# TongkunGuan/CCD

Measured on AMD Instinct MI355X. Metric: images/sec (32x128 crops, 2 views) CCD-ViT-Small pretrain step, higher is better.
Workload: dtype bf16; 1 GPU; CCD_pretrain_vit_small bf16, bs=256/GPU, 2 views 32x128, out_dim=65536, drop_path 0.1, dataset-mask branch (pseudo-epoch 1), synthetic batch in HBM; global_batch=256, parallelism=dp1

## Files before the change

### ccd_amd/csrc/abi_impl.h

```cpp
#pragma once

#include "../../include/ccd_hip.h"
#include "kernels/common.h"
#include "kernels/gemm.h"
#include "kernels/gemm256.h"
#include "kernels/gemm_row384.h"
#include "kernels/mlp_fused.h"
#include "kernels/rowgemm.h"
#include "kernels/mlp_bwd.h"
#include "kernels/rowproj.h"
#include "kernels/attention_fwd.h"
#include "kernels/attention_probs.h"
#include "kernels/attention_bwd.h"
#include "kernels/attention_bwd1.h"
#include "kernels/gemm_tn384.h"
#include "kernels/layernorm.h"
#include "kernels/charmap.h"
#include "kernels/cluster.h"
#include "kernels/ssim.h"
#include "kernels/datapipe.h"
#include "kernels/embed.h"
#include "kernels/head.h"
#include "kernels/loss.h"
#include "kernels/headloss.h"
#include "kernels/optim.h"
#include "kernels/conv.h"
#include "kernels/cls_tail.h"
#include "kernels/decoder.h"
#include "kernels/decoder_xattn.h"

#define CCD_CHECK(cond, code) \
    do {                      \
        if (!(cond)) return (code); \
    } while (0)
#define CCD_ALIGNED16(p) ((((uintptr_t)(p)) & 15u) == 0)
#define CCD_MAX_OPERAND_BYTES 0x7ffffff0L

static int ccd_grid_cus(long tiles = 0);
static int ccd_gemm_grid(ccd::GemmParams& p, int tiles, int splits) {
    p.work_items = tiles * splits;
    const int cap = 2 * ccd_grid_cus((p.work_items + 1) / 2);
    return p.work_items < cap ? p.work_items : cap;
}

template <bool TN>
static int ccd_launch_gemm(ccd::GemmParams p, int epilogue, int splits, void* stream) {
    const int tiles = ((p.M + ccd::GEMM_BM - 1) / ccd::GEMM_BM) * ((p.N + ccd::GEMM_BN - 1) / ccd::GEMM_BN);
    const dim3 grid(ccd_gemm_grid(p, tiles, splits)), block(256);
    const size_t smem = ccd::GEMM_SMEM_BYTES;
    switch (epilogue) {
        case CCD_EPI_BF16: CCD_LAUNCH((ccd::gemm_bf16_kernel<TN, ccd::EPI_BF16>), grid, block, smem, stream, p); break;
        case CCD_EPI_GELU: CCD_LAUNCH((ccd::gemm_bf16_kernel<TN, ccd::EPI_GELU>), grid, block, smem, stream, p); break;
        case CCD_EPI_RESID: CCD_LAUNCH((ccd::gemm_bf16_kernel<TN, ccd::EPI_RESID>), grid, block, smem, stream, p); break;
        case CCD_EPI_F32: CCD_LAUNCH((ccd::gemm_bf16_kernel<TN, ccd::EPI_F32>), grid, block, smem, stream, p); break;
        case CCD_EPI_ATOMIC: CCD_LAUNCH((ccd::gemm_bf16_kernel<TN, ccd::EPI_ATOMIC>), grid, block, smem, stream, p); break;
        case CCD_EPI_DGELU: CCD_LAUNCH((ccd::gemm_bf16_kernel<TN, ccd::EPI_DGELU>), grid, block, smem, stream, p); break;
        default: return CCD_EINVAL;
    }
    return ccd_rt_last_error();
}

static unsigned ccd_stream_blocks(long total, int per_thread) {
    long blocks = (total + 256L * per_thread - 1) / (256L * per_thread);
    const long cap = 16L * ccd_rt_num_cus();
    if (blocks > cap) blocks = cap;
    return (unsigned)(blocks < 1 ? 1 : blocks);
}
static void ccd_reduce_geometry(long rows, int N, int* cgn_log2, int* col_blocks, int* rows_per_block, int* row_blocks) {
    int lg = 0;
    while (lg < 5 && (8 << lg) < N) ++lg;
    const int cgn = 1 << lg, rln = ccd::COLSUM_THREADS >> lg;
    *cgn_log2 = lg;
    *col_blocks = (N + 8 * cgn - 1) / (8 * cgn);
    long rb = (rows * (long)(16 * cgn) + (1L << 17) - 1) / (1L << 17);
    const long cap = (2L * ccd_rt_num_cus() + *col_blocks - 1) / *col_blocks;
    if (rb > cap) rb = cap;
    if (rb < 1) rb = 1;
    long rpb = (rows + rb - 1) / rb;
    rpb = ((rpb + rln - 1) / rln) * rln;
    *rows_per_block = (int)rpb;
    *row_blocks = (int)((rows + rpb - 1) / rpb);
}
struct CcdPolicy {
    int gemm_256 = 1;
    int gemm_256_min_m = 2048, gemm_256_min_n = 384;
    int gemm_256_f32 = 0;
    int gemm_256_deep = 0;
    int gemm_row384 = 0;
    int rowproj = 1;
    int rowproj_min_m = 16384;
    int rowproj_rb = 0;
    int rowgemm = 1;
    int ln_bwd_bpc = 5;
    int dec_attn_simt = 0;
    int attn_tr = 1;
    int attn_onepass = 1;
    int attn_skew = 0;
    int gemm_tn384 = 1;
    int gemm_tn384_geom = 0;
    int gemm_tn384_min_tiles = 6;
    int cu_reserve = 0;
    int cu_reserve_window = -1;
    int cu_reserve_left = 0;
    int rowgemm_adma = 1;
    int tn_ws = 1;
    int lab = 0;
};
struct CcdPolicyKey { const char* name; int CcdPolicy::*field; };
static const CcdPolicyKey ccd_policy_keys[] = {
    {"gemm_256", &CcdPolicy::gemm_256}, {"gemm_256_min_m", &CcdPolicy::gemm_256_min_m},
    {"gemm_256_min_n", &CcdPolicy::gemm_256_min_n}, {"gemm_256_f32", &CcdPolicy::gemm_256_f32},
    {"gemm_256_deep", &CcdPolicy::gemm_256_deep}, {"gemm_row384", &CcdPolicy::gemm_row384},
    {"rowproj", &CcdPolicy::rowproj}, {"rowproj_min_m", &CcdPolicy::rowproj_min_m}, {"rowproj_rb", &CcdPolicy::rowproj_rb},
    {"rowgemm", &CcdPolicy::rowgemm}, {"ln_bwd_bpc", &CcdPolicy::ln_bwd_bpc}, {"dec_attn_simt", &CcdPolicy::dec_attn_simt}, {"attn_onepass", &CcdPolicy::attn_onepass}, {"attn_skew", &CcdPolicy::attn_skew}, {"attn_tr", &CcdPolicy::attn_tr}, {"gemm_tn384", &CcdPolicy::gemm_tn384}, {"gemm_tn384_min_tiles", &CcdPolicy::gemm_tn384_min_tiles}, {"gemm_tn384_geom", &CcdPolicy::gemm_tn384_geom}, {"cu_reserve", &CcdPolicy::cu_reserve}, {"cu_reserve_window", &CcdPolicy::cu_reserve_window}, {"cu_reserve_left", &CcdPolicy::cu_reserve_left}, {"rowgemm_adma", &CcdPolicy::rowgemm_adma}, {"tn_ws", &CcdPolicy::tn_ws}, {"lab", &CcdPolicy::lab}};
static CcdPolicy& ccd_policy() {
    static CcdPolicy pol = [] {
        CcdPolicy q;
        for (const CcdPolicyKey& k : ccd_policy_keys) {
            char env[64] = "CCD_";
            size_t n = 4;
            for (const char* c = k.name; *c && n + 1 < sizeof(env); ++c) env[n++] = (char)(*c >= 'a' && *c <= 'z' ? *c - 32 : *c);
            env[n] = 0;
            if (const char* v = getenv(env)) q.*(k.field) = atoi(v);
        }
        return q;
    }();
    return pol;
}
static int ccd_grid_cus(long tiles) {
    CcdPolicy& pol = ccd_policy();
    int reserve = pol.cu_reserve;
    if (reserve > 0 && pol.cu_reserve_window >= 0) {
        if (pol.cu_reserve_left > 0) --pol.cu_reserve_left;
        else reserve = 0;
    }
    const int all = ccd_rt_num_cus();
    if (reserve > 0 && tiles > 0 && 8 * reserve <= all) {
        const long full = (tiles + all - 1) / all, less = (tiles + (all - reserve) - 1) / (all - reserve);
        if (less > full && full <= 4) reserve = 0;
    }
    const int cus = all - reserve;
    return cus > 1 ? cus : 1;
}
static bool ccd_rowproj_takes(const ccd::GemmParams& p, int epilogue) {
    const CcdPolicy& pol = ccd_policy();
    return pol.rowproj && epilogue == CCD_EPI_BF16 && (p.K == 384 || p.K == 512) && p.N % 64 == 0 && p.N <= 4096 &&
           p.M >= pol.rowproj_min_m && !p.d_rows && !p.colsum && p.alpha == 1.0f && p.ldc % 8 == 0 &&
           ccd::rp_smem_bytes(p.K, p.N) <= 160 * 1024 &&
           ((long)p.M + 512) * p.lda * 2 < CCD_MAX_OPERAND_BYTES && ((long)p.M + 512) * p.ldc * 2 < CCD_MAX_OPERAND_BYTES;
}
static int ccd_launch_rowproj(const ccd::GemmParams& p, void* stream) {
    ccd::RowProjParams q;
    q.a = reinterpret_cast<const ccd::bf16_t*>(p.A); q.lda = p.lda; q.w = reinterpret_cast<const ccd::bf16_t*>(p.B); q.ldw = p.ldb;
    q.bias = p.bias; q.out = reinterpret_cast<ccd::bf16_t*>(p.C); q.ldc = p.ldc; q.M = p.M; q.N = p.N;
    const int cus = ccd_grid_cus((p.M + ccd::rp_rows(p.K == 384 ? 2 : 1) - 1) / ccd::rp_rows(p.K == 384 ? 2 : 1)), smem = ccd::rp_smem_bytes(p.K, p.N);
    if (p.K == 384) {
        const int tiles = (p.M + ccd::rp_rows(2) - 1) / ccd::rp_rows(2), rb = ccd_policy().rowproj_rb;
        if (rb == 1 || (rb == 0 && tiles < cus)) {
            const int tiles1 = (p.M + ccd::rp_rows(1) - 1) / ccd::rp_rows(1);
            CCD_LAUNCH((ccd::rowproj_kernel<384, 1>), dim3(tiles1 < cus ? tiles1 : cus), dim3(ccd::RP_THREADS), smem, stream, q);
        } else {
            CCD_LAUNCH((ccd::rowproj_kernel<384, 2>), dim3(tiles < cus ? tiles : cus), dim3(ccd::RP_THREADS), smem, stream, q);
        }
    } else {
        const int tiles = (p.M + ccd::rp_rows(1) - 1) / ccd::rp_rows(1);
        CCD_LAUNCH((ccd::rowproj_kernel<512, 1>), dim3(tiles < cus ? tiles : cus), dim3(ccd::RP_THREADS), smem, stream, q);
    }
    return ccd_rt_last_error();
}
template <int BN, bool DEEP = false>
static int ccd_launch_gemm256(const ccd::GemmParams& p, int epilogue, void* stream) {
    const int tiles = ((p.M + ccd::G256_BM - 1) / ccd::G256_BM) * ((p.N + BN - 1) / BN);
    const int cus = ccd_grid_cus();
    const dim3 grid(tiles < cus ? tiles : cus), block(ccd::G256_THREADS);
    const size_t smem = ccd::g256_smem_bytes(p.N, p.colsum != nullptr);
    switch (epilogue) {
        case CCD_EPI_BF16: CCD_LAUNCH((ccd::gemm256_kernel<ccd::EPI_BF16, BN, DEEP>), grid, block, smem, stream, p); break;
        case CCD_EPI_GELU: CCD_LAUNCH((ccd::gemm256_kernel<ccd::EPI_GELU, BN, DEEP>), grid, block, smem, stream, p); break;
        case CCD_EPI_RESID: CCD_LAUNCH((ccd::gemm256_kernel<ccd::EPI_RESID, BN, DEEP>), grid, block, smem, stream, p); break;
        case CCD_EPI_F32: CCD_LAUNCH((ccd::gemm256_kernel<ccd::EPI_F32, BN, DEEP>), grid, block, smem, stream, p); break;
        case CCD_EPI_DGELU: CCD_LAUNCH((ccd::gemm256_kernel<ccd::EPI_DGELU, BN, DEEP>), grid, block, smem, stream, p); break;
        default: return CCD_EINVAL;
    }
    return ccd_rt_last_error();
}
static int ccd_launch_gemm_row384(const ccd::GemmParams& p, int epilogue, void* stream, int cus = -1) {
    const int tiles = (p.M + ccd::GR_BM - 1) / ccd::GR_BM;
    if (cus < 0) cus = ccd_grid_cus(tiles);
    const dim3 grid(tiles < cus ? tiles : cus), block(ccd::GR_THREADS);
    const size_t smem = ccd::GR_SMEM_BYTES;
    switch (epilogue) {
        case CCD_EPI_BF16: CCD_LAUNCH((ccd::gemm_row384_kernel<ccd::EPI_BF16>), grid, block, smem, stream, p); break;
        case CCD_EPI_RESID: CCD_LAUNCH((ccd::gemm_row384_kernel<ccd::EPI_RESID>), grid, block, smem, stream, p); break;
        case CCD_EPI_F32: CCD_LAUNCH((ccd::gemm_row384_kernel<ccd::EPI_F32>), grid, block, smem, stream, p); break;
        case 7: CCD_LAUNCH((ccd::gemm_row384_kernel<ccd::EPI_RESID_LN>), grid, block, smem, stream, p); break;
        case 8: CCD_LAUNCH((ccd::gemm_row384_kernel<ccd::EPI_LNBWD>), grid, block, smem, stream, p); break;
        default: return CCD_EINVAL;
    }
    return ccd_rt_last_error();
}

template <int WM, int WN, int STAGES, int TI, int TJ>
static int ccd_launch_tn384_geom(ccd::GemmParams& p, int Mc, float* ws, long ws_floats, void* stream) {
    using G = ccd::Tn3Geom<WM, WN, STAGES, TI, TJ>;
    const int per_cu = 8 / G::WAVES;
    const int t1 = (p.M / G::TP) * (p.N / G::TQ), t2 = (p.M2 / G::TP) * (p.N2 / G::TQ), slots = per_cu * ccd_grid_cus();
    const int xcds = slots >= 8 * (t1 > t2 ? t1 : t2) ? 8 : 1;
    const int spx = slots / xcds;
    int s1 = 0, s2 = 0;
    unsigned long long units1 = 0, units2 = 0;
    for (int x = 0; x < xcds; ++x) {
        int rem = spx, u1 = 0, u2 = 0;
        while (true) {
            const bool first = t2 == 0 || s1 < s2 || (s1 == s2 && t1 >= t2);
            if (first && t1 <= rem && u1 < 255) { ++u1; ++s1; rem -= t1; }
            else if (!first && t2 <= rem && u2 < 255) { ++u2; ++s2; rem -= t2; }
            else if (first && t2 > 0 && s2 <= s1 && t2 <= rem && u2 < 255) { ++u2; ++s2; rem -= t2; }
            else if (!first && s1 <= s2 && t1 <= rem && u1 < 255) { ++u1; ++s1; rem -= t1; }
            else break;
        }
        units1 |= (unsigned long long)u1 << (8 * x);
        units2 |= (unsigned long long)u2 << (8 * x);
    }
    if (s1 < 1 || (t2 > 0 && s2 < 1)) return CCD_ESHAPE;
    auto rows_per = [&](int& slices) {
        int per = (Mc + slices - 1) / slices;
        per = ((per + ccd::TN3_BK - 1) / ccd::TN3_BK) * ccd::TN3_BK;
        slices = (Mc + per - 1) / per;
        return per;
    };
    p.k_per_split = rows_per(s1); p.work_items = s1;
    if (t2 > 0) { p.per2 = rows_per(s2); p.slices2 = s2; }
    p.units1 = units1; p.units2 = units2; p.m_fastest = xcds;
    const long need1 = (long)s1 * p.M * p.N, need2 = t2 > 0 ? (long)s2 * p.M2 * p.N2 : 0;
    const bool use_ws = ws && need1 + need2 <= ws_floats && (s1 > 1 || s2 > 1) && p.ldc % 4 == 0 && (t2 == 0 || p.ldc2 % 4 == 0) &&
                        !(p.rps_shift & 1);
    p.ws = use_ws ? ws : nullptr;
    p.ws2 = use_ws ? ws + need1 : nullptr;
    CCD_LAUNCH((ccd::gemm_tn384_kernel<WM, WN, STAGES, TI, TJ>), dim3(xcds * spx), dim3(G::THREADS), G::SMEM_BYTES, stream, p);
    if (use_ws) {
        ccd::Tn3ReduceParams r;
        r.ws[0] = p.ws; r.ws[1] = p.ws2; r.C[0] = reinterpret_cast<float*>(p.C); r.C[1] = reinterpret_cast<float*>(p.C2);
        r.ldc[0] = p.ldc; r.ldc[1] = p.ldc2; r.S[0] = s1; r.S[1] = t2 > 0 ? s2 : 0; r.P[0] = p.M; r.P[1] = t2 > 0 ? p.M2 : 0;
        r.Q[0] = p.N; r.Q[1] = t2 > 0 ? p.N2 : 0; r.alpha = p.alpha;
        const long n4 = ((long)p.M * p.N + (t2 > 0 ? (long)p.M2 * p.N2 : 0)) / 4;
        CCD_LAUNCH(ccd::tn3_reduce_kernel, dim3((unsigned)((n4 + 255) / 256)), dim3(256), 0, stream, r);
    }
    return ccd_rt_last_error();
}

extern "C" {

int ccd_abi_version(void) { return 16; }
const char* ccd_build_info(void) { return "ccd_hip gfx950 bf16-mfma abi16"; }
int ccd_policy_set(const char* key, int value) {
    CCD_CHECK(key, CCD_EINVAL);
    for (const CcdPolicyKey& k : ccd_policy_keys)
        if (!strcmp(k.name, key)) { ccd_policy().*(k.field) = value; return CCD_OK; }
    return CCD_EINVAL;
}
int ccd_policy_get(const char* key, int* value) {
    CCD_CHECK(key && value, CCD_EINVAL);
    for (const CcdPolicyKey& k : ccd_policy_keys)
        if (!strcmp(k.name, key)) { *value = ccd_policy().*(k.field); return CCD_OK; }
    return CCD_EINVAL;
}

int ccd_gemm_nt(const ccd_bf16* A, long lda, const ccd_bf16* B, long ldb, int M, int N, int K, int epilogue, void* C,
                long ldc, void* C2, long ldc2, const float* bias, const float* resid, long ldr,
                const float* rowscale, int rows_per_sample, const ccd_bf16* aux, long ldaux, float alpha,
                int m_fastest, const int* d_rows, int rows_mul, float* colsum, void* stream) {
    CCD_CHECK(A && B && (C || (epilogue == CCD_EPI_GELU && C2)), CCD_EINVAL);
    CCD_CHECK(CCD_ALIGNED16(A) && CCD_ALIGNED16(B) && CCD_ALIGNED16(C), CCD_EINVAL);
    CCD_CHECK(!colsum || epilogue == CCD_EPI_BF16 || epilogue == CCD_EPI_DGELU, CCD_EINVAL);
    if (M == 0 || N == 0) return CCD_OK;
    CCD_CHECK(M > 0 && N > 0 && K > 0, CCD_EINVAL);
    CCD_CHECK(K % 64 == 0 && N % 8 == 0 && lda % 8 == 0 && ldb % 8 == 0 && ldc % 4 == 0, CCD_ESHAPE);
    CCD_CHECK(((long)M * lda + K) * 2 < CCD_MAX_OPERAND_BYTES && ((long)N * ldb + K) * 2 < CCD_MAX_OPERAND_BYTES, CCD_ESHAPE);
    CCD_CHECK(epilogue != CCD_EPI_GELU || (C2 && ldc2 % 8 == 0), CCD_EINVAL);
    CCD_CHECK(epilogue != CCD_EPI_RESID || (resid && ldr % 4 == 0 && rows_per_sample > 0), CCD_EINVAL);
    CCD_CHECK(epilogue != CCD_EPI_DGELU || (aux && ldaux % 8 == 0 && (!C2 || ldc2 % 8 == 0)), CCD_EINVAL);
    ccd::GemmParams p = ccd::GemmParams();
    p.A = A; p.B = B; p.lda = lda; p.ldb = ldb; p.M = M; p.N = N; p.K = K;
    p.C = C; p.ldc = ldc; p.C2 = C2; p.ldc2 = ldc2; p.bias = bias; p.resid = resid; p.ldr = ldr;
    p.rowscale = rowscale; p.rows_per_sample = rows_per_sample; p.aux = aux; p.ldaux = ldaux;
    p.rps_shift = -1;
    if (rows_per_sample > 0 && (rows_per_sample & (rows_per_sample - 1)) == 0)
        for (int sft = 0; sft < 31; ++sft) if ((1 << sft) == rows_per_sample) p.rps_shift = sft;
    p.k_per_split = K; p.m_fastest = m_fastest; p.alpha = alpha; p.d_rows = d_rows; p.rows_mul = rows_mul;
    p.colsum = colsum;
    const CcdPolicy& pol = ccd_policy();
    if (ccd_rowproj_takes(p, epilogue)) return ccd_launch_rowproj(p, stream);
    if (pol.gemm_row384 >= 1 && N <= ccd::GR_BN && M >= pol.gemm_256_min_m &&
        (epilogue == CCD_EPI_RESID || epilogue == CCD_EPI_F32 || (epilogue == CCD_EPI_BF16 && pol.gemm_row384 >= 2)))
        return ccd_launch_gemm_row384(p, epilogue, stream);
    const bool bf16_out = epilogue == CCD_EPI_BF16 || epilogue == CCD_EPI_GELU || epilogue == CCD_EPI_DGELU;
    const bool f32_256 = epilogue != CCD_EPI_ATOMIC && (pol.gemm_256_f32 || N % 256 == 0);
    const bool colsum_fits = !colsum || N <= ccd::G256_MAX_COLSUM_N;
    const bool dgelu_fits = epilogue != CCD_EPI_DGELU || (((long)M + 256) * ldaux * 2 < CCD_MAX_OPERAND_BYTES &&
        ((long)M + 256) * ldc * 2 < CCD_MAX_OPERAND_BYTES && (!C2 || ((long)M + 256) * ldc2 * 2 < CCD_MAX_OPERAND_BYTES));
    if (pol.gemm_256 >= 1 && (bf16_out || f32_256) && M >= pol.gemm_256_min_m &&
        N >= pol.gemm_256_min_n && colsum_fits && dgelu_fits) {
        if (pol.gemm_256_deep) return ccd_launch_gemm256<256, true>(p, epilogue, stream);
        return ccd_launch_gemm256<256>(p, epilogue, stream);
    }
    if (pol.gemm_256 >= 2 && epilogue != CCD_EPI_ATOMIC && M >= pol.gemm_256_min_m && colsum_fits && dgelu_fits) return ccd_launch_gemm256<128>(p, epilogue, stream);
    int splits = 1;
    if (epilogue == CCD_EPI_ATOMIC && K >= 16384) {
        p.k_per_split = 8192;
        splits = (K + 8191) / 8192;
    }
    return ccd_launch_gemm<false>(p, epilogue, splits, stream);
}

int ccd_gemm_nt_resid_ln(const ccd_bf16* A, long lda, const ccd_bf16* B, long ldb, int M, int N, int K, float* C, long ldc,
                         const float* bias, const float* resid, long ldr, const float* rowscale, int rows_per_sample,
                         const float* ln_gamma, const float* ln_beta, float ln_eps, ccd_bf16* y, long ldy, float* mean,
                         float* rstd, void* stream) {
    CCD_CHECK(A && B && C && resid && ln_gamma && ln_beta && y && mean && rstd, CCD_EINVAL);
    CCD_CHECK(CCD_ALIGNED16(A) && CCD_ALIGNED16(B) && CCD_ALIGNED16(C) && CCD_ALIGNED16(resid) && CCD_ALIGNED16(y), CCD_EINVAL);
    if (M == 0) return CCD_OK;
    CCD_CHECK(M > 0 && N > 0 && K > 0 && rows_per_sample > 0, CCD_EINVAL);
    CCD_CHECK(N <= 512 && N % 8 == 0 && K % 64 == 0 && lda % 8 == 0 && ldb % 8 == 0 && ldc % 4 == 0 && ldr % 4 == 0 &&
              ldy % 8 == 0, CCD_ESHAPE);
    CCD_CHECK(((long)M * lda + K) * 2 < CCD_MAX_OPERAND_BYTES && ((long)N * ldb + K) * 2 < CCD_MAX_OPERAND_BYTES, CCD_ESHAPE);
    const int cus = ccd_grid_cus((M + ccd::RG_BM - 1) / ccd::RG_BM);
    if (ccd_policy().rowgemm && (N == 512 || ccd_policy().rowgemm == 2) && (N == 128 || N == 256 || N == 384 || N == 512) &&
        K % (64 * ccd::rg_ring(N)) == 0 &&
        ((long)M + (long)cus * ccd::RG_BM) * lda * 2 < CCD_MAX_OPERAND_BYTES && (long)M * ldr * 4 < CCD_MAX_OPERAND_BYTES &&
        (long)M * ldc * 4 < CCD_MAX_OPERAND_BYTES) {
        ccd::RowGemmParams q = ccd::RowGemmParams();
        q.A = A; q.lda = lda; q.W = B; q.ldw = ldb; q.M = M; q.K = K; q.gamma = ln_gamma; q.ln_beta = ln_beta; q.ln_eps = ln_eps;
        q.bias = bias; q.resid = resid; q.ldr = ldr; q.out = C; q.ldc = ldc; q.ln_y = y; q.ld_y = ldy; q.ln_mean = mean;
        q.ln_rstd = rstd; q.rowscale = rowscale; q.rows_per_sample = rows_per_sample; q.lab = ccd_policy().lab;
        const int tiles = (M + ccd::RG_BM - 1) / ccd::RG_BM, smem = ccd::rg_smem_bytes(N);
        const dim3 grid(tiles < cus ? tiles : cus), block(ccd::RG_THREADS);
        if (N == 512) CCD_LAUNCH((ccd::rowgemm_kernel<512, ccd::rg_ring(512), ccd::RG_RESID_LN>), grid, block, smem, stream, q);
        else if (N == 384 && ccd_policy().rowgemm_adma)
            CCD_LAUNCH((ccd::rowgemm_kernel<384, 3, ccd::RG_RESID_LN, true>), grid, block, ccd::rg_smem_bytes_adma(384), stream, q);
        else if (N == 384) CCD_LAUNCH((ccd::rowgemm_kernel<384, ccd::rg_ring(384), ccd::RG_RESID_LN>), grid, block, smem, stream, q);
        else if (N == 256) CCD_LAUNCH((ccd::rowgemm_kernel<256, ccd::rg_ring(256), ccd::RG_RESID_LN>), grid, block, smem, stream, q);
        else CCD_LAUNCH((ccd::rowgemm_kernel<128, ccd::rg_ring(128), ccd::RG_RESID_LN>), grid, block, smem, stream, q);
        return ccd_rt_last_error();
    }
    CCD_CHECK(N <= ccd::GR_BN, CCD_ESHAPE);
    ccd::GemmParams p = ccd::GemmParams();
    p.A = A; p.B = B; p.lda = lda; p.ldb = ldb; p.M = M; p.N = N; p.K = K; p.C = C; p.ldc = ldc; p.bias = bias;
    p.resid = resid; p.ldr = ldr; p.rowscale = rowscale; p.rows_per_sample = rows_per_sample; p.alpha = 1.0f; p.rows_mul = 1;
    p.k_per_split = K;
    p.rps_shift = -1;
    for (int sft = 0; sft < 31; ++sft) if ((1 << sft) == rows_per_sample) p.rps_shift = sft;
    p.ln_gamma = ln_gamma; p.ln_beta = ln_beta; p.ln_eps = ln_eps; p.ln_y = y; p.ld_y = ldy; p.ln_mean = mean; p.ln_rstd = rstd;
    return ccd_launch_gemm_row384(p, 7 , stream, cus);
}

struct CcdLnTap {
    const ccd_bf16* tap_dy = nullptr;
    long ld_tap = 0;
    const float* tap_gamma = nullptr;
    float* tap_dgamma = nullptr;
    float* tap_dbeta = nullptr;
};
static int ccd_gemm_nt_lnbwd_any(const ccd_bf16* A, long lda, const ccd_bf16* B, long ldb, int M, int N, int K, const float* x, long ldx,
                                 const float* mean, const float* rstd, const float* gamma, void* g, int g16, long ldg, int accumulate,
                                 float* dgamma, float* dbeta, ccd_bf16* gb, long ldgb, const float* rowscale, int rows_per_sample,
                                 float* dbias, void* stream, const CcdLnTap& tap = CcdLnTap()) {
    if (tap.tap_dy) {
        CCD_CHECK(tap.tap_gamma && tap.tap_dgamma && tap.tap_dbeta && CCD_ALIGNED16(tap.tap_dy) && tap.ld_tap % 8 == 0, CCD_EINVAL);
        CCD_CHECK(g16 && N == 384 && ccd_policy().rowgemm && K % (64 * ccd::rg_ring(N)) == 0 && (long)M * tap.ld_tap * 2 < CCD_MAX_OPERAND_BYTES,
                  CCD_ESHAPE);
    }
    CCD_CHECK(A && B && x && mean && rstd && gamma && g && dgamma && dbeta, CCD_EINVAL);
    CCD_CHECK(CCD_ALIGNED16(A) && CCD_ALIGNED16(B) && CCD_ALIGNED16(x) && CCD_ALIGNED16(g) && CCD_ALIGNED16(gb), CCD_EINVAL);
    if (M == 0) return CCD_OK;
    CCD_CHECK(M > 0 && N > 0 && K > 0 && (!rowscale || rows_per_sample > 0), CCD_EINVAL);
    CCD_CHECK(N <= 512 && N % 8 == 0 && K % 64 == 0 && lda % 8 == 0 && ldb % 8 == 0 && ldx % 4 == 0 && ldg % 4 == 0 &&
              (!gb || ldgb % 4 == 0), CCD_ESHAPE);
    CCD_CHECK(((long)M * lda + K) * 2 < CCD_MAX_OPERAND_BYTES && ((long)N * ldb + K) * 2 < CCD_MAX_OPERAND_BYTES, CCD_ESHAPE);
    const int cus = ccd_grid_cus((M + ccd::RG_BM - 1) / ccd::RG_BM);
    if (ccd_policy().rowgemm && (N == 128 || N == 256 || N == 384 || N == 512) && K % (64 * ccd::rg_ring(N)) == 0 && ldg % 4 == 0 &&
        ((long)M + (long)cus * ccd::RG_BM) * lda * 2 < CCD_MAX_OPERAND_BYTES && (long)M * ldx * 4 < CCD_MAX_OPERAND_BYTES &&
        (long)M * ldg * 4 < CCD_MAX_OPERAND_BYTES && (!g16 || (N <= 384 && ldg % 8 == 0))) {
        ccd::RowGemmParams q;
        q.A = A; q.lda = lda; q.W = B; q.ldw = ldb; q.M = M; q.K = K; q.x = x; q.ldx = ldx; q.mean = mean; q.rstd = rstd;
        q.gamma = gamma; q.g = g; q.ldg = ldg; q.accumulate = accumulate; q.dgamma = dgamma; q.dbeta = dbeta; q.gb = gb;
        q.ld_gb = ldgb; q.rowscale = gb ? rowscale : nullptr; q.rows_per_sample = rows_per_sample > 0 ? rows_per_sample : 1;
        q.dbias = gb ? dbias : nullptr; q.lab = ccd_policy().lab;
        q.bias = nullptr; q.resid = nullptr; q.out = nullptr; q.ln_beta = nullptr; q.ln_y = nullptr; q.ln_mean = q.ln_rstd = nullptr;
        q.ldr = q.ldc = q.ld_y = 0; q.ln_eps = 0.f;
        q.tap_dy = tap.tap_dy; q.ld_tap = tap.ld_tap; q.tap_gamma = tap.tap_gamma; q.tap_dgamma = tap.tap_dgamma; q.tap_dbeta = tap.tap_dbeta;
        const int tiles = (M + ccd::RG_BM - 1) / ccd::RG_BM, smem = ccd::rg_smem_bytes(N);
        const dim3 grid(tiles < cus ? tiles : cus), block(ccd::RG_THREADS);
// ... 1356 lines not shown
```

### ccd_amd/csrc/kernels/gemm_tn384.h

```cpp
#pragma once

namespace ccd {

constexpr int TN3_BK = 32;
template <int WM, int WN, int STAGES_, int TI_ = 3, int TJ_ = 3>
struct Tn3Geom {
    static constexpr int WAVES = WM * WN, THREADS = 64 * WAVES, STAGES = STAGES_, TI = TI_, TJ = TJ_;
    static constexpr int TP = 32 * TI * WM, TQ = 32 * TJ * WN;
    static constexpr int A_ROWB = TP * 2, B_ROWB = TQ * 2;
    static constexpr int A_BYTES = TN3_BK * A_ROWB, B_BYTES = TN3_BK * B_ROWB, STAGE_BYTES = A_BYTES + B_BYTES;
    static constexpr int SMEM_BYTES = STAGES * STAGE_BYTES;
    static constexpr int A_PIECES = A_BYTES / 1024 / WAVES;
    static constexpr int B_TOTAL = B_BYTES / 1024;
    static constexpr int B_PIECES = (B_TOTAL + WAVES - 1) / WAVES;
    static constexpr int B_FULL = B_TOTAL - (B_PIECES - 1) * WAVES;
    static constexpr int PER_STAGE = A_PIECES + B_PIECES;
    static_assert((TI == 3 && TJ == 3) || (TI == 4 && TJ == 2), "the two hand-scheduled stage bodies below");
    static_assert(A_BYTES % (1024 * WAVES) == 0 && (PER_STAGE == 5 || PER_STAGE == 6), "piece schedule below");
};
template <int ROWB>
__device__ __forceinline__ int tn3_swz(int row) {
    static_assert(ROWB % 256 == 0 || ROWB % 256 == 128, "");
    return ROWB % 256 == 0 ? (row & 3) << 2 : ((row >> 1) & 1) << 2;
}

template <int WM, int WN, int STAGES, int TI = 3, int TJ = 3>
__global__ __launch_bounds__(64 * WM * WN, 8 / (WM * WN)) void gemm_tn384_kernel(GemmParams p) {
    using G = Tn3Geom<WM, WN, STAGES, TI, TJ>;
    constexpr int AHEAD = STAGES - 1;
    char* smem = dynamic_smem();
    const int t = threadIdx.x, lane = t & 63, w = t >> 6, hf = lane >> 5, lq = lane & 31;
    const int wm = w % WM, wn = w / WM;
    const int tiles1 = (p.M / G::TP) * (p.N / G::TQ), tiles2 = (p.M2 / G::TP) * (p.N2 / G::TQ);
    const int xcds = p.m_fastest, xcd = (int)blockIdx.x % xcds, slot = (int)blockIdx.x / xcds;
    const int u1 = (int)((p.units1 >> (8 * xcd)) & 255ull), u2 = (int)((p.units2 >> (8 * xcd)) & 255ull);
    int base1 = 0, base2 = 0;
    for (int y = 0; y < xcd; ++y) {
        base1 += (int)((p.units1 >> (8 * y)) & 255ull);
        base2 += (int)((p.units2 >> (8 * y)) & 255ull);
    }
    int tile, slice;
    if (slot < u1 * tiles1) {
        tile = slot % tiles1;
        slice = base1 + slot / tiles1;
    } else {
        const int s2 = slot - u1 * tiles1;
        if (s2 >= u2 * tiles2) return;
        tile = s2 % tiles2;
        slice = base2 + s2 / tiles2;
        p.A = p.A2; p.B = p.B2; p.lda = p.lda2; p.ldb = p.ldb2; p.M = p.M2; p.N = p.N2; p.C = p.C2; p.ldc = p.ldc2;
        p.k_per_split = p.per2; p.work_items = p.slices2; p.ws = p.ws2;
    }
    if (slice >= p.work_items) return;
    const int tiles_q = p.N / G::TQ;
    const int p0 = (tile / tiles_q) * G::TP, q0 = (tile % tiles_q) * G::TQ;
    const int k_begin = slice * p.k_per_split;
    const int k_end = k_begin + p.k_per_split < p.K ? k_begin + p.k_per_split : p.K;
    const int nk = k_end > k_begin ? (k_end - k_begin) / TN3_BK : 0;
    if (nk == 0) return;

    const bf16_t* ga[G::A_PIECES];
    const bf16_t* gb[G::B_PIECES];
#pragma unroll
    for (int i = 0; i < G::A_PIECES; ++i) {
        const int byte = 1024 * (G::A_PIECES * w + i) + 16 * lane;
        const int row = byte / G::A_ROWB, pos = (byte % G::A_ROWB) >> 4;
        ga[i] = p.A + (long)(k_begin + row) * p.lda + p0 + (pos ^ tn3_swz<G::A_ROWB>(row)) * 8;
    }
#pragma unroll
    for (int i = 0; i < G::B_PIECES; ++i) {
        const int byte = 1024 * (w + G::WAVES * i) + 16 * lane;
        const int row = (byte / G::B_ROWB) & (TN3_BK - 1), pos = (byte % G::B_ROWB) >> 4;
        gb[i] = p.B + (long)(k_begin + row) * p.ldb + q0 + (pos ^ tn3_swz<G::B_ROWB>(row)) * 8;
    }
    const long a_step = (long)TN3_BK * p.lda, b_step = (long)TN3_BK * p.ldb;
    const bool b_last = w < G::B_FULL;
    auto dma_piece = [&](int s, int i) {
        char* base = smem + (s % STAGES) * G::STAGE_BYTES;
        if (i < G::A_PIECES) {
            stream_glds16<NT_TN>(ga[i], base + (G::A_PIECES * w + i) * 1024);
            ga[i] += a_step;
        } else {
            const int ib = i - G::A_PIECES;
            if (ib < G::B_PIECES - 1 || b_last) {
                stream_glds16<NT_TN>(gb[ib], base + G::A_BYTES + (w + G::WAVES * ib) * 1024);
                gb[ib] += b_step;
            }
        }
    };
    auto dma = [&](int s) {
#pragma unroll
        for (int i = 0; i < G::PER_STAGE; ++i) dma_piece(s, i);
    };
    auto wait_steps = [&](int in_flight) {
        if (b_last) {
            if (in_flight >= 3) glds_wait<3 * G::PER_STAGE>();
            else if (in_flight == 2) glds_wait<2 * G::PER_STAGE>();
            else if (in_flight == 1) glds_wait<G::PER_STAGE>();
            else glds_wait_all();
        } else {
            if (in_flight >= 3) glds_wait<3 * (G::PER_STAGE - 1)>();
            else if (in_flight == 2) glds_wait<2 * (G::PER_STAGE - 1)>();
            else if (in_flight == 1) glds_wait<G::PER_STAGE - 1>();
            else glds_wait_all();
        }
    };

    const int j = lane & 15, g16 = (lane >> 4) & 1, r4 = j >> 2, c4 = j & 3;
    unsigned base_a[TI], base_b[TJ];
    {
        const int row = 8 * hf + r4;
#pragma unroll
        for (int i = 0; i < TI; ++i) {
            const int chunk_a = 4 * TI * wm + 4 * i + 2 * g16 + (c4 >> 1);
            base_a[i] = (unsigned)(row * G::A_ROWB + ((chunk_a ^ tn3_swz<G::A_ROWB>(row)) << 4) + (c4 & 1) * 8);
        }
#pragma unroll
        for (int i = 0; i < TJ; ++i) {
            const int chunk_b = 4 * TJ * wn + 4 * i + 2 * g16 + (c4 >> 1);
            base_b[i] = (unsigned)(G::A_BYTES + row * G::B_ROWB + ((chunk_b ^ tn3_swz<G::B_ROWB>(row)) << 4) + (c4 & 1) * 8);
        }
    }

    const unsigned smem_addr = lds_addr_of(smem);
    f32x16 acc[TI][TJ];
#pragma unroll
    for (int i = 0; i < TI; ++i)
#pragma unroll
        for (int jj = 0; jj < TJ; ++jj)
#pragma unroll
            for (int r = 0; r < 16; ++r) acc[i][jj][r] = 0.f;

#ifdef CCD_MLP_LAB
    unsigned long long ph[6] = {0, 0, 0, 0, 0, 0};
    unsigned long long tprev = __builtin_amdgcn_s_memtime();
#define TN3_STAMP(i) if (p.rps_shift & 4) { const unsigned long long tn_ = __builtin_amdgcn_s_memtime(); ph[i] += tn_ - tprev; tprev = tn_; }
#else
#define TN3_STAMP(i)
#endif
#pragma unroll
    for (int s = 0; s < AHEAD; ++s)
        if (s < nk) dma(s);
    wait_steps((nk < AHEAD ? nk : AHEAD) - 1);
    lds_barrier();
    for (int kt = 0; kt < ((p.rps_shift & 2) ? 1 : nk); ++kt) {
        const bool more = kt + AHEAD < nk && !(p.rps_shift & 8);
        TN3_STAMP(0)
        const unsigned sb = smem_addr + (unsigned)((kt % STAGES) * G::STAGE_BYTES);
        const unsigned aa0 = sb + base_a[0], aa1 = sb + base_a[1], aa2 = sb + base_a[2], aa3 = sb + base_a[TI - 1];
        const unsigned ab0 = sb + base_b[0], ab1 = sb + base_b[1], ab2 = sb + base_b[TJ - 1];
        tr_u32x2 x[2][6][2];
#define TN3_RD_A(ks, slot, addr)                                                     \
        lds_read_tr<(16 * ks) * G::A_ROWB>(x[ks][slot][0], addr);                       \
        lds_read_tr<(16 * ks + 4) * G::A_ROWB>(x[ks][slot][1], addr);
#define TN3_RD_B(ks, slot, addr)                                                     \
        lds_read_tr<(16 * ks) * G::B_ROWB>(x[ks][slot][0], addr);                       \
        lds_read_tr<(16 * ks + 4) * G::B_ROWB>(x[ks][slot][1], addr);
#define TN3_FRAG(ks, slot) frag_from_tr(x[ks][slot][0], x[ks][slot][1])
        if constexpr (TI == 3) {
        TN3_RD_A(0, 0, aa0) TN3_RD_B(0, 1, ab0) TN3_RD_B(0, 2, ab1) TN3_RD_B(0, 3, ab2) TN3_RD_A(0, 4, aa1) TN3_RD_A(0, 5, aa2)
        bf16x8 a0 = TN3_FRAG(0, 0), b0 = TN3_FRAG(0, 1), b1 = TN3_FRAG(0, 2), b2 = TN3_FRAG(0, 3), a1 = TN3_FRAG(0, 4), a2 = TN3_FRAG(0, 5);
        lds_wait_frag<8>(b0);
        TN3_STAMP(1)
        acc[0][0] = mfma_32x32x16_bf16(a0, b0, acc[0][0]);
        lds_wait_frag<6>(b1);
        acc[0][1] = mfma_32x32x16_bf16(a0, b1, acc[0][1]);
        lds_wait_frag<4>(b2);
        acc[0][2] = mfma_32x32x16_bf16(a0, b2, acc[0][2]);
        CCD_SCHED_FENCE();
        if (more) dma_piece(kt + AHEAD, 0);
        CCD_SCHED_FENCE();
        TN3_RD_A(1, 0, aa0) TN3_RD_B(1, 1, ab0)
        lds_wait_frag<6>(a1);
        acc[1][0] = mfma_32x32x16_bf16(a1, b0, acc[1][0]);
        acc[1][1] = mfma_32x32x16_bf16(a1, b1, acc[1][1]);
        acc[1][2] = mfma_32x32x16_bf16(a1, b2, acc[1][2]);
        CCD_SCHED_FENCE();
        if (more) dma_piece(kt + AHEAD, 1);
        CCD_SCHED_FENCE();
        TN3_RD_B(1, 2, ab1) TN3_RD_B(1, 3, ab2)
        lds_wait_frag<8>(a2);
        acc[2][0] = mfma_32x32x16_bf16(a2, b0, acc[2][0]);
        acc[2][1] = mfma_32x32x16_bf16(a2, b1, acc[2][1]);
        acc[2][2] = mfma_32x32x16_bf16(a2, b2, acc[2][2]);
        CCD_SCHED_FENCE();
        if (more) dma_piece(kt + AHEAD, 2);
        CCD_SCHED_FENCE();
        TN3_RD_A(1, 4, aa1) TN3_RD_A(1, 5, aa2)
        a0 = TN3_FRAG(1, 0); b0 = TN3_FRAG(1, 1); b1 = TN3_FRAG(1, 2); b2 = TN3_FRAG(1, 3); a1 = TN3_FRAG(1, 4); a2 = TN3_FRAG(1, 5);
        lds_wait_frag<8>(b0);
        acc[0][0] = mfma_32x32x16_bf16(a0, b0, acc[0][0]);
        lds_wait_frag<6>(b1);
        acc[0][1] = mfma_32x32x16_bf16(a0, b1, acc[0][1]);
        lds_wait_frag<4>(b2);
        acc[0][2] = mfma_32x32x16_bf16(a0, b2, acc[0][2]);
        CCD_SCHED_FENCE();
        if (more) dma_piece(kt + AHEAD, 3);
        CCD_SCHED_FENCE();
        lds_wait_frag<2>(a1);
        acc[1][0] = mfma_32x32x16_bf16(a1, b0, acc[1][0]);
        acc[1][1] = mfma_32x32x16_bf16(a1, b1, acc[1][1]);
        acc[1][2] = mfma_32x32x16_bf16(a1, b2, acc[1][2]);
        CCD_SCHED_FENCE();
        if (more) dma_piece(kt + AHEAD, 4);
        CCD_SCHED_FENCE();
        lds_wait_frag<0>(a2);
        acc[2][0] = mfma_32x32x16_bf16(a2, b0, acc[2][0]);
        acc[2][1] = mfma_32x32x16_bf16(a2, b1, acc[2][1]);
        acc[2][2] = mfma_32x32x16_bf16(a2, b2, acc[2][2]);
        } else {
        TN3_RD_A(0, 0, aa0) TN3_RD_B(0, 1, ab0) TN3_RD_B(0, 2, ab1) TN3_RD_A(0, 3, aa1) TN3_RD_A(0, 4, aa2) TN3_RD_A(0, 5, aa3)
        bf16x8 a0 = TN3_FRAG(0, 0), b0 = TN3_FRAG(0, 1), b1 = TN3_FRAG(0, 2), a1 = TN3_FRAG(0, 3), a2 = TN3_FRAG(0, 4), a3 = TN3_FRAG(0, 5);
        lds_wait_frag<8>(b0);
        TN3_STAMP(1)
        acc[0][0] = mfma_32x32x16_bf16(a0, b0, acc[0][0]);
        lds_wait_frag<6>(b1);
        acc[0][1] = mfma_32x32x16_bf16(a0, b1, acc[0][1]);
        CCD_SCHED_FENCE();
        if (more) dma_piece(kt + AHEAD, 0);
        CCD_SCHED_FENCE();
        TN3_RD_A(1, 0, aa0) TN3_RD_B(1, 1, ab0)
        lds_wait_frag<8>(a1);
        acc[1][0] = mfma_32x32x16_bf16(a1, b0, acc[1][0]);
        acc[1][1] = mfma_32x32x16_bf16(a1, b1, acc[1][1]);
        CCD_SCHED_FENCE();
        if (more) dma_piece(kt + AHEAD, 1);
        CCD_SCHED_FENCE();
        TN3_RD_B(1, 2, ab1) TN3_RD_A(1, 3, aa1)
        lds_wait_frag<10>(a2);
        acc[2][0] = mfma_32x32x16_bf16(a2, b0, acc[2][0]);
        acc[2][1] = mfma_32x32x16_bf16(a2, b1, acc[2][1]);
        CCD_SCHED_FENCE();
        if (more) dma_piece(kt + AHEAD, 2);
        CCD_SCHED_FENCE();
        TN3_RD_A(1, 4, aa2) TN3_RD_A(1, 5, aa3)
        lds_wait_frag<12>(a3);
        acc[3][0] = mfma_32x32x16_bf16(a3, b0, acc[3][0]);
        acc[3][1] = mfma_32x32x16_bf16(a3, b1, acc[3][1]);
        a0 = TN3_FRAG(1, 0); b0 = TN3_FRAG(1, 1); b1 = TN3_FRAG(1, 2); a1 = TN3_FRAG(1, 3); a2 = TN3_FRAG(1, 4); a3 = TN3_FRAG(1, 5);
        lds_wait_frag<8>(b0);
        acc[0][0] = mfma_32x32x16_bf16(a0, b0, acc[0][0]);
        lds_wait_frag<6>(b1);
        acc[0][1] = mfma_32x32x16_bf16(a0, b1, acc[0][1]);
        CCD_SCHED_FENCE();
        if (more) dma_piece(kt + AHEAD, 3);
        CCD_SCHED_FENCE();
        lds_wait_frag<4>(a1);
        acc[1][0] = mfma_32x32x16_bf16(a1, b0, acc[1][0]);
        acc[1][1] = mfma_32x32x16_bf16(a1, b1, acc[1][1]);
        CCD_SCHED_FENCE();
        if (more) dma_piece(kt + AHEAD, 4);
        CCD_SCHED_FENCE();
        lds_wait_frag<2>(a2);
        acc[2][0] = mfma_32x32x16_bf16(a2, b0, acc[2][0]);
        acc[2][1] = mfma_32x32x16_bf16(a2, b1, acc[2][1]);
        lds_wait_frag<0>(a3);
        acc[3][0] = mfma_32x32x16_bf16(a3, b0, acc[3][0]);
        acc[3][1] = mfma_32x32x16_bf16(a3, b1, acc[3][1]);
        }
#undef TN3_RD_A
#undef TN3_RD_B
#undef TN3_FRAG
        if (G::PER_STAGE == 6) {
            CCD_SCHED_FENCE();
            if (more) dma_piece(kt + AHEAD, 5);
        }
        TN3_STAMP(2)
        const int rem = nk - 1 - kt;
        if (rem > 0) wait_steps((rem < AHEAD ? rem : AHEAD) - 1);
        TN3_STAMP(3)
        if (!(p.rps_shift & 16)) lds_barrier();
        TN3_STAMP(4)
    }
#ifdef CCD_MLP_LAB
    if ((p.rps_shift & 4) && p.colsum_a && blockIdx.x < 32 && lane == 0 && (w == 0 || w == G::WAVES - 1)) {
        unsigned long long* o = reinterpret_cast<unsigned long long*>(p.colsum_a) + (blockIdx.x * 2 + (w ? 1 : 0)) * 6;
        for (int i = 0; i < 6; ++i) o[i] = ph[i];
    }
#endif
    glds_wait_all();

    float* C = reinterpret_cast<float*>(p.C);
    if (p.rps_shift & 1) return;
    if (p.ws) {
        float* W = p.ws + (long)slice * p.M * p.N;
#pragma unroll
        for (int i = 0; i < TI; ++i)
#pragma unroll
            for (int jj = 0; jj < TJ; ++jj) {
                float* cp = W + (long)(p0 + 32 * TI * wm + 32 * i + 4 * hf) * p.N + (q0 + 32 * TJ * wn + 32 * jj + lq);
#pragma unroll
                for (int r = 0; r < 16; ++r) cp[(long)((r & 3) + 8 * (r >> 2)) * p.N] = acc[i][jj][r];
            }
        return;
    }
#pragma unroll
    for (int i = 0; i < TI; ++i)
#pragma unroll
        for (int jj = 0; jj < TJ; ++jj) {
            float* cp = C + (long)(p0 + 32 * TI * wm + 32 * i + 4 * hf) * p.ldc + (q0 + 32 * TJ * wn + 32 * jj + lq);
#pragma unroll
            for (int r = 0; r < 16; ++r) atomicAdd(cp + (long)((r & 3) + 8 * (r >> 2)) * p.ldc, acc[i][jj][r] * p.alpha);
        }
}

struct Tn3ReduceParams {
    const float* ws[2];
    float* C[2];
    long ldc[2];
    int S[2], P[2], Q[2];
    float alpha;
};
__global__ __launch_bounds__(256) void tn3_reduce_kernel(Tn3ReduceParams p) {
    const long n0 = (long)p.P[0] * p.Q[0] / 4, n1 = (long)p.P[1] * p.Q[1] / 4;
    long i = (long)blockIdx.x * 256 + threadIdx.x;
    int which = 0;
    if (i >= n0) { i -= n0; which = 1; if (i >= n1) return; }
    const long plane = (long)p.P[which] * p.Q[which];
    const float* src = p.ws[which] + 4 * i;
    f32x4v s = {0.f, 0.f, 0.f, 0.f};
    const int S = p.S[which];
    int k = 0;
    for (; k + 4 <= S; k += 4) {
        const f32x4v a = *reinterpret_cast<const f32x4v*>(src + (long)k * plane), b = *reinterpret_cast<const f32x4v*>(src + (long)(k + 1) * plane);
        const f32x4v c = *reinterpret_cast<const f32x4v*>(src + (long)(k + 2) * plane), d = *reinterpret_cast<const f32x4v*>(src + (long)(k + 3) * plane);
        s.x += (a.x + b.x) + (c.x + d.x); s.y += (a.y + b.y) + (c.y + d.y); s.z += (a.z + b.z) + (c.z + d.z); s.w += (a.w + b.w) + (c.w + d.w);
    }
    for (; k < S; ++k) {
        const f32x4v a = *reinterpret_cast<const f32x4v*>(src + (long)k * plane);
        s.x += a.x; s.y += a.y; s.z += a.z; s.w += a.w;
    }
    const long e = 4 * i, row = e / p.Q[which], col = e % p.Q[which];
    float* dst = p.C[which] + row * p.ldc[which] + col;
    f32x4v o = *reinterpret_cast<f32x4v*>(dst);
    o.x += p.alpha * s.x; o.y += p.alpha * s.y; o.z += p.alpha * s.z; o.w += p.alpha * s.w;
    *reinterpret_cast<f32x4v*>(dst) = o;
}

}
```

Baseline: 5344 images/sec.

## Add 16x16x32 MFMA variant of the TN weight-gradient GEMM kernel

Adds an alternate stage body for the 96x96-per-wave TN GEMM that uses 16x16x32 bf16 MFMA instructions instead of the 32x32 variant. It comes with a new LDS swizzle, fragment addressing, and an interleaved schedule of LDS reads, MFMAs and DMA pieces. A transposed-accumulator option lets the workspace path write contiguous f32x4 stores. It is selected by default through a new policy knob. The aim is better MFMA issue and LDS-read overlap, at the cost of more MFMA instructions and a different register footprint.

```diff
diff --git a/ccd_amd/csrc/abi_impl.h b/ccd_amd/csrc/abi_impl.h
--- a/ccd_amd/csrc/abi_impl.h
+++ b/ccd_amd/csrc/abi_impl.h
@@ -98,6 +98,7 @@
     int attn_skew = 0;
     int gemm_tn384 = 1;
     int gemm_tn384_geom = 0;
+    int gemm_tn384_mfma = 16;
     int gemm_tn384_min_tiles = 6;
     int cu_reserve = 0;
     int cu_reserve_window = -1;
@@ -112,7 +113,7 @@
     {"gemm_256_min_n", &CcdPolicy::gemm_256_min_n}, {"gemm_256_f32", &CcdPolicy::gemm_256_f32},
     {"gemm_256_deep", &CcdPolicy::gemm_256_deep}, {"gemm_row384", &CcdPolicy::gemm_row384},
     {"rowproj", &CcdPolicy::rowproj}, {"rowproj_min_m", &CcdPolicy::rowproj_min_m}, {"rowproj_rb", &CcdPolicy::rowproj_rb},
-    {"rowgemm", &CcdPolicy::rowgemm}, {"ln_bwd_bpc", &CcdPolicy::ln_bwd_bpc}, {"dec_attn_simt", &CcdPolicy::dec_attn_simt}, {"attn_onepass", &CcdPolicy::attn_onepass}, {"attn_skew", &CcdPolicy::attn_skew}, {"attn_tr", &CcdPolicy::attn_tr}, {"gemm_tn384", &CcdPolicy::gemm_tn384}, {"gemm_tn384_min_tiles", &CcdPolicy::gemm_tn384_min_tiles}, {"gemm_tn384_geom", &CcdPolicy::gemm_tn384_geom}, {"cu_reserve", &CcdPolicy::cu_reserve}, {"cu_reserve_window", &CcdPolicy::cu_reserve_window}, {"cu_reserve_left", &CcdPolicy::cu_reserve_left}, {"rowgemm_adma", &CcdPolicy::rowgemm_adma}, {"tn_ws", &CcdPolicy::tn_ws}, {"lab", &CcdPolicy::lab}};
+    {"rowgemm", &CcdPolicy::rowgemm}, {"ln_bwd_bpc", &CcdPolicy::ln_bwd_bpc}, {"dec_attn_simt", &CcdPolicy::dec_attn_simt}, {"attn_onepass", &CcdPolicy::attn_onepass}, {"attn_skew", &CcdPolicy::attn_skew}, {"attn_tr", &CcdPolicy::attn_tr}, {"gemm_tn384", &CcdPolicy::gemm_tn384}, {"gemm_tn384_min_tiles", &CcdPolicy::gemm_tn384_min_tiles}, {"gemm_tn384_geom", &CcdPolicy::gemm_tn384_geom}, {"gemm_tn384_mfma", &CcdPolicy::gemm_tn384_mfma}, {"cu_reserve", &CcdPolicy::cu_reserve}, {"cu_reserve_window", &CcdPolicy::cu_reserve_window}, {"cu_reserve_left", &CcdPolicy::cu_reserve_left}, {"rowgemm_adma", &CcdPolicy::rowgemm_adma}, {"tn_ws", &CcdPolicy::tn_ws}, {"lab", &CcdPolicy::lab}};
 static CcdPolicy& ccd_policy() {
     static CcdPolicy pol = [] {
         CcdPolicy q;
@@ -237,7 +238,14 @@
                         !(p.rps_shift & 1);
     p.ws = use_ws ? ws : nullptr;
     p.ws2 = use_ws ? ws + need1 : nullptr;
-    CCD_LAUNCH((ccd::gemm_tn384_kernel<WM, WN, STAGES, TI, TJ>), dim3(xcds * spx), dim3(G::THREADS), G::SMEM_BYTES, stream, p);
+    if constexpr (TI == 3 && TJ == 3) {
+        if (ccd_policy().gemm_tn384_mfma == 16)
+            CCD_LAUNCH((ccd::gemm_tn384_mfma16_kernel<WM, WN, STAGES>), dim3(xcds * spx), dim3(G::THREADS), G::SMEM_BYTES, stream, p);
+        else
+            CCD_LAUNCH((ccd::gemm_tn384_kernel<WM, WN, STAGES, TI, TJ>), dim3(xcds * spx), dim3(G::THREADS), G::SMEM_BYTES, stream, p);
+    } else {
+        CCD_LAUNCH((ccd::gemm_tn384_kernel<WM, WN, STAGES, TI, TJ>), dim3(xcds * spx), dim3(G::THREADS), G::SMEM_BYTES, stream, p);
+    }
     if (use_ws) {
         ccd::Tn3ReduceParams r;
         r.ws[0] = p.ws; r.ws[1] = p.ws2; r.C[0] = reinterpret_cast<float*>(p.C); r.C[1] = reinterpret_cast<float*>(p.C2);
diff --git a/ccd_amd/csrc/kernels/gemm_tn384.h b/ccd_amd/csrc/kernels/gemm_tn384.h
--- a/ccd_amd/csrc/kernels/gemm_tn384.h
+++ b/ccd_amd/csrc/kernels/gemm_tn384.h
@@ -18,15 +18,19 @@
     static_assert((TI == 3 && TJ == 3) || (TI == 4 && TJ == 2), "the two hand-scheduled stage bodies below");
     static_assert(A_BYTES % (1024 * WAVES) == 0 && (PER_STAGE == 5 || PER_STAGE == 6), "piece schedule below");
 };
-template <int ROWB>
+template <int ROWB, int MF = 32>
 __device__ __forceinline__ int tn3_swz(int row) {
     static_assert(ROWB % 256 == 0 || ROWB % 256 == 128, "");
+    if (MF == 16) return ROWB % 256 == 0 ? ((row & 3) << 1) | (((row >> 3) & 1) << 3) : (((row >> 1) & 1) << 1) | (((row >> 3) & 1) << 2);
     return ROWB % 256 == 0 ? (row & 3) << 2 : ((row >> 1) & 1) << 2;
 }
 
-template <int WM, int WN, int STAGES, int TI = 3, int TJ = 3>
-__global__ __launch_bounds__(64 * WM * WN, 8 / (WM * WN)) void gemm_tn384_kernel(GemmParams p) {
+template <bool B>
+struct Tn3Tag { static constexpr bool value = B; };
+template <int WM, int WN, int STAGES, int TI, int TJ, int MF>
+__device__ __forceinline__ void tn3_body(GemmParams p) {
     using G = Tn3Geom<WM, WN, STAGES, TI, TJ>;
+    static_assert(MF == 32 || (MF == 16 && TI == 3 && TJ == 3), "the 16x16x32 stage body is written for 96 x 96 per wave");
     constexpr int AHEAD = STAGES - 1;
     char* smem = dynamic_smem();
     const int t = threadIdx.x, lane = t & 63, w = t >> 6, hf = lane >> 5, lq = lane & 31;
@@ -65,13 +69,13 @@
     for (int i = 0; i < G::A_PIECES; ++i) {
         const int byte = 1024 * (G::A_PIECES * w + i) + 16 * lane;
         const int row = byte / G::A_ROWB, pos = (byte % G::A_ROWB) >> 4;
-        ga[i] = p.A + (long)(k_begin + row) * p.lda + p0 + (pos ^ tn3_swz<G::A_ROWB>(row)) * 8;
+        ga[i] = p.A + (long)(k_begin + row) * p.lda + p0 + (pos ^ tn3_swz<G::A_ROWB, MF>(row)) * 8;
     }
 #pragma unroll
     for (int i = 0; i < G::B_PIECES; ++i) {
         const int byte = 1024 * (w + G::WAVES * i) + 16 * lane;
         const int row = (byte / G::B_ROWB) & (TN3_BK - 1), pos = (byte % G::B_ROWB) >> 4;
-        gb[i] = p.B + (long)(k_begin + row) * p.ldb + q0 + (pos ^ tn3_swz<G::B_ROWB>(row)) * 8;
+        gb[i] = p.B + (long)(k_begin + row) * p.ldb + q0 + (pos ^ tn3_swz<G::B_ROWB, MF>(row)) * 8;
     }
     const long a_step = (long)TN3_BK * p.lda, b_step = (long)TN3_BK * p.ldb;
     const bool b_last = w < G::B_FULL;
@@ -106,31 +110,6 @@
         }
     };
 
-    const int j = lane & 15, g16 = (lane >> 4) & 1, r4 = j >> 2, c4 = j & 3;
-    unsigned base_a[TI], base_b[TJ];
-    {
-        const int row = 8 * hf + r4;
-#pragma unroll
-        for (int i = 0; i < TI; ++i) {
-            const int chunk_a = 4 * TI * wm + 4 * i + 2 * g16 + (c4 >> 1);
-            base_a[i] = (unsigned)(row * G::A_ROWB + ((chunk_a ^ tn3_swz<G::A_ROWB>(row)) << 4) + (c4 & 1) * 8);
-        }
-#pragma unroll
-        for (int i = 0; i < TJ; ++i) {
-            const int chunk_b = 4 * TJ * wn + 4 * i + 2 * g16 + (c4 >> 1);
-            base_b[i] = (unsigned)(G::A_BYTES + row * G::B_ROWB + ((chunk_b ^ tn3_swz<G::B_ROWB>(row)) << 4) + (c4 & 1) * 8);
-        }
-    }
-
-    const unsigned smem_addr = lds_addr_of(smem);
-    f32x16 acc[TI][TJ];
-#pragma unroll
-    for (int i = 0; i < TI; ++i)
-#pragma unroll
-        for (int jj = 0; jj < TJ; ++jj)
-#pragma unroll
-            for (int r = 0; r < 16; ++r) acc[i][jj][r] = 0.f;
-
 #ifdef CCD_MLP_LAB
     unsigned long long ph[6] = {0, 0, 0, 0, 0, 0};
     unsigned long long tprev = __builtin_amdgcn_s_memtime();
@@ -138,6 +117,175 @@
 #else
 #define TN3_STAMP(i)
 #endif
+    if constexpr (MF == 16) {
+        const int i16 = lane & 15, kg = lane >> 4, r4 = i16 >> 2, c4 = i16 & 3, row = 8 * kg + r4;
+        const unsigned smem_addr = lds_addr_of(smem);
+        unsigned fa[6], fb[6];
+#pragma unroll
+        for (int i = 0; i < 6; ++i) {
+            const int chunk_a = 12 * wm + 2 * i + (c4 >> 1), chunk_b = 12 * wn + 2 * i + (c4 >> 1);
+            fa[i] = (unsigned)(row * G::A_ROWB + ((chunk_a ^ tn3_swz<G::A_ROWB, 16>(row)) << 4) + (c4 & 1) * 8);
+            fb[i] = (unsigned)(G::A_BYTES + row * G::B_ROWB + ((chunk_b ^ tn3_swz<G::B_ROWB, 16>(row)) << 4) + (c4 & 1) * 8);
+        }
+        const bool tr_acc = (p.ws != nullptr) != ((p.rps_shift & 32) != 0);
+        auto run16 = [&](auto tr_tag) {
+        constexpr bool TR = decltype(tr_tag)::value;
+        f32x4 acc[6][6];
+#pragma unroll
+        for (int i = 0; i < 6; ++i)
+#pragma unroll
+            for (int jj = 0; jj < 6; ++jj) acc[i][jj] = f32x4{0.f, 0.f, 0.f, 0.f};
+#pragma unroll
+        for (int s = 0; s < AHEAD; ++s)
+            if (s < nk) dma(s);
+        wait_steps((nk < AHEAD ? nk : AHEAD) - 1);
+        lds_barrier();
+        for (int kt = 0; kt < ((p.rps_shift & 2) ? 1 : nk); ++kt) {
+            const bool more = kt + AHEAD < nk && !(p.rps_shift & 8);
+            TN3_STAMP(0)
+            const unsigned sb = smem_addr + (unsigned)((kt % STAGES) * G::STAGE_BYTES);
+            tr_u32x2 xa[6][2], xb[6][2];
+#define TN3_RD16_A(i) lds_read_tr<0>(xa[i][0], sb + fa[i]); lds_read_tr<4 * G::A_ROWB>(xa[i][1], sb + fa[i]);
+#define TN3_RD16_B(i) lds_read_tr<0>(xb[i][0], sb + fb[i]); lds_read_tr<4 * G::B_ROWB>(xb[i][1], sb + fb[i]);
+#define TN3_MM16(i, jj, a, b) acc[i][jj] = TR ? mfma_16x16x32_bf16(b, a, acc[i][jj]) : mfma_16x16x32_bf16(a, b, acc[i][jj]);
+#define TN3_ROW16(i)                                                                                              \
+            TN3_MM16(i, 0, a##i, b0) TN3_MM16(i, 1, a##i, b1) \
+            TN3_MM16(i, 2, a##i, b2) TN3_MM16(i, 3, a##i, b3) \
+            TN3_MM16(i, 4, a##i, b4) TN3_MM16(i, 5, a##i, b5)
+            TN3_RD16_A(0) TN3_RD16_B(0) TN3_RD16_B(1) TN3_RD16_B(2) TN3_RD16_B(3) TN3_RD16_B(4) TN3_RD16_B(5)
+            bf16x8 a0 = frag_from_tr(xa[0][0], xa[0][1]), b0 = frag_from_tr(xb[0][0], xb[0][1]), b1 = frag_from_tr(xb[1][0], xb[1][1]);
+            bf16x8 b2 = frag_from_tr(xb[2][0], xb[2][1]), b3 = frag_from_tr(xb[3][0], xb[3][1]), b4 = frag_from_tr(xb[4][0], xb[4][1]);
+            bf16x8 b5 = frag_from_tr(xb[5][0], xb[5][1]);
+            lds_wait_frag<10>(b0);
+            TN3_STAMP(1)
+            TN3_MM16(0, 0, a0, b0)
+            lds_wait_frag<8>(b1);
+            TN3_MM16(0, 1, a0, b1)
+            lds_wait_frag<6>(b2);
+            TN3_MM16(0, 2, a0, b2)
+            CCD_SCHED_FENCE();
+            if (more) dma_piece(kt + AHEAD, 0);
+            CCD_SCHED_FENCE();
+            TN3_RD16_A(1) TN3_RD16_A(2)
+            bf16x8 a1 = frag_from_tr(xa[1][0], xa[1][1]), a2 = frag_from_tr(xa[2][0], xa[2][1]);
+            lds_wait_frag<8>(b3);
+            TN3_MM16(0, 3, a0, b3)
+            lds_wait_frag<6>(b4);
+            TN3_MM16(0, 4, a0, b4)
+            lds_wait_frag<4>(b5);
+            TN3_MM16(0, 5, a0, b5)
+            CCD_SCHED_FENCE();
+            if (more) dma_piece(kt + AHEAD, 1);
+            CCD_SCHED_FENCE();
+            TN3_RD16_A(3) TN3_RD16_A(4)
+            bf16x8 a3 = frag_from_tr(xa[3][0], xa[3][1]), a4 = frag_from_tr(xa[4][0], xa[4][1]);
+            lds_wait_frag<6>(a1);
+            TN3_ROW16(1)
+            CCD_SCHED_FENCE();
+            if (more) dma_piece(kt + AHEAD, 2);
+            CCD_SCHED_FENCE();
+            TN3_RD16_A(5)
+            bf16x8 a5 = frag_from_tr(xa[5][0], xa[5][1]);
+            lds_wait_frag<6>(a2);
+            TN3_ROW16(2)
+            CCD_SCHED_FENCE();
+            if (more) dma_piece(kt + AHEAD, 3);
+            CCD_SCHED_FENCE();
+            lds_wait_frag<4>(a3);
+            TN3_ROW16(3)
+            CCD_SCHED_FENCE();
+            if (more) dma_piece(kt + AHEAD, 4);
+            CCD_SCHED_FENCE();
+            lds_wait_frag<2>(a4);
+            TN3_ROW16(4)
+            if (G::PER_STAGE == 6) {
+                CCD_SCHED_FENCE();
+                if (more) dma_piece(kt + AHEAD, 5);
+                CCD_SCHED_FENCE();
+            }
+            lds_wait_frag<0>(a5);
+            TN3_ROW16(5)
+#undef TN3_RD16_A
+#undef TN3_RD16_B
+#undef TN3_ROW16
+#undef TN3_MM16
+            TN3_STAMP(2)
+            const int rem = nk - 1 - kt;
+            if (rem > 0) wait_steps((rem < AHEAD ? rem : AHEAD) - 1);
+            TN3_STAMP(3)
+            if (!(p.rps_shift & 16)) lds_barrier();
+            TN3_STAMP(4)
+        }
+#ifdef CCD_MLP_LAB
+        if ((p.rps_shift & 4) && p.colsum_a && blockIdx.x < 32 && lane == 0 && (w == 0 || w == G::WAVES - 1)) {
+            unsigned long long* o = reinterpret_cast<unsigned long long*>(p.colsum_a) + (blockIdx.x * 2 + (w ? 1 : 0)) * 6;
+            for (int i = 0; i < 6; ++i) o[i] = ph[i];
+        }
+#endif
+        glds_wait_all();
+        if (p.rps_shift & 1) return;
+        if (TR) {
+            const int prow = p0 + 96 * wm + i16, qcol = q0 + 96 * wn + 4 * kg;
+            if (p.ws) {
+                float* W = p.ws + (long)slice * p.M * p.N;
+#pragma unroll
+                for (int i = 0; i < 6; ++i)
+#pragma unroll
+                    for (int jj = 0; jj < 6; ++jj)
+                        *reinterpret_cast<f32x4*>(W + (long)(prow + 16 * i) * p.N + (qcol + 16 * jj)) = acc[i][jj];
+                return;
+            }
+#pragma unroll
+            for (int i = 0; i < 6; ++i)
+#pragma unroll
+                for (int jj = 0; jj < 6; ++jj) {
+                    float* cp = reinterpret_cast<float*>(p.C) + (long)(prow + 16 * i) * p.ldc + (qcol + 16 * jj);
+#pragma unroll
+                    for (int r = 0; r < 4; ++r) atomicAdd(cp + r, acc[i][jj][r] * p.alpha);
+                }
+        } else {
+            const int prow = p0 + 96 * wm + 4 * kg, qcol = q0 + 96 * wn + i16;
+            float* W = p.ws ? p.ws + (long)slice * p.M * p.N : nullptr;
+#pragma unroll
+            for (int i = 0; i < 6; ++i)
+#pragma unroll
+                for (int jj = 0; jj < 6; ++jj)
+#pragma unroll
+                    for (int r = 0; r < 4; ++r) {
+                        if (W) W[(long)(prow + 16 * i + r) * p.N + (qcol + 16 * jj)] = acc[i][jj][r];
+                        else atomicAdd(reinterpret_cast<float*>(p.C) + (long)(prow + 16 * i + r) * p.ldc + (qcol + 16 * jj), acc[i][jj][r] * p.alpha);
+                    }
+        }
+        };
+        if (tr_acc) run16(Tn3Tag<true>{});
+        else run16(Tn3Tag<false>{});
+        return;
+    } else {
+    const int j = lane & 15, g16 = (lane >> 4) & 1, r4 = j >> 2, c4 = j & 3;
+    unsigned base_a[TI], base_b[TJ];
+    {
+        const int row = 8 * hf + r4;
+#pragma unroll
+        for (int i = 0; i < TI; ++i) {
+            const int chunk_a = 4 * TI * wm + 4 * i + 2 * g16 + (c4 >> 1);
+            base_a[i] = (unsigned)(row * G::A_ROWB + ((chunk_a ^ tn3_swz<G::A_ROWB, MF>(row)) << 4) + (c4 & 1) * 8);
+        }
+#pragma unroll
+        for (int i = 0; i < TJ; ++i) {
+            const int chunk_b = 4 * TJ * wn + 4 * i + 2 * g16 + (c4 >> 1);
+            base_b[i] = (unsigned)(G::A_BYTES + row * G::B_ROWB + ((chunk_b ^ tn3_swz<G::B_ROWB, MF>(row)) << 4) + (c4 & 1) * 8);
+        }
+    }
+
+    const unsigned smem_addr = lds_addr_of(smem);
+    f32x16 acc[TI][TJ];
+#pragma unroll
+    for (int i = 0; i < TI; ++i)
+#pragma unroll
+        for (int jj = 0; jj < TJ; ++jj)
+#pragma unroll
+            for (int r = 0; r < 16; ++r) acc[i][jj][r] = 0.f;
+
 #pragma unroll
     for (int s = 0; s < AHEAD; ++s)
         if (s < nk) dma(s);
@@ -302,6 +450,15 @@
 #pragma unroll
             for (int r = 0; r < 16; ++r) atomicAdd(cp + (long)((r & 3) + 8 * (r >> 2)) * p.ldc, acc[i][jj][r] * p.alpha);
         }
+    }
+}
+template <int WM, int WN, int STAGES, int TI = 3, int TJ = 3>
+__global__ __launch_bounds__(64 * WM * WN, 8 / (WM * WN)) void gemm_tn384_kernel(GemmParams p) {
+    tn3_body<WM, WN, STAGES, TI, TJ, 32>(p);
+}
+template <int WM, int WN, int STAGES>
+__global__ __launch_bounds__(64 * WM * WN, 8 / (WM * WN)) void gemm_tn384_mfma16_kernel(GemmParams p) {
+    tn3_body<WM, WN, STAGES, 3, 3, 16>(p);
 }
 
 struct Tn3ReduceParams {
```

New measurement: 5375 images/sec, median of 6. No clear change (+0.6%).
